# marvinli00/genie2

Measured on AMD Instinct MI355X. Metric: denoise-steps/sec (N=256, T=1000, batch=8), higher is better.
Workload: dtype f32 (pair-stack products as 3 f16 MFMAs on 2xf16-split operands, f32 accumulate); 1 GPU; unconditional N=256, T=1000, batch=8 per GPU, random-init base Denoiser (15.7M params), scale=0.6, reverse-loop steps 995..667; parallelism=replica per GPU x1, no data-path collective

## Files before the change

### genie2_amd/capi.py

```python
import ctypes as C
import os

import torch

_HERE = os.path.dirname(os.path.abspath(__file__))
LIB_PATH = os.environ.get('GENIE_HIP_LIB', os.path.join(_HERE, 'lib', 'libgenie_hip.so'))


class GenieDims(C.Structure):
    _fields_ = [
        ('c_s', C.c_int32), ('c_p', C.c_int32),
        ('c_pos_emb', C.c_int32), ('c_chain_emb', C.c_int32), ('c_timestep_emb', C.c_int32),
        ('relpos_k', C.c_int32),
        ('template_dist_n_bin', C.c_int32),
        ('template_dist_min', C.c_float), ('template_dist_step', C.c_float),
        ('n_pair_transform_layer', C.c_int32), ('c_hidden_mul', C.c_int32), ('pair_transition_n', C.c_int32),
        ('n_structure_layer', C.c_int32), ('n_structure_block', C.c_int32),
        ('c_hidden_ipa', C.c_int32), ('n_head_ipa', C.c_int32), ('n_qk_point', C.c_int32), ('n_v_point', C.c_int32),
        ('rescale', C.c_float),
        ('n_timestep', C.c_int32), ('max_n_res', C.c_int32), ('max_n_chain', C.c_int32),
    ]


class GenieFeatures(C.Structure):
    _fields_ = [(k, C.c_void_p) for k in (
        'aatype', 'atom_positions', 'residue_mask', 'residue_index', 'chain_index',
        'fixed_sequence_mask', 'fixed_structure_mask', 'interface_mask')]


class GenieTaps(C.Structure):
    _fields_ = [(k, C.c_void_p) for k in ('s', 'p', 's_final', 'rots_out', 'trans_out', 'p_init', 'p_layer0', 'states', 'p_trimul_out0',
                                              'ipa_cat0')]


class GenieGemmDesc(C.Structure):
    _fields_ = [(n, C.c_int32) for n in ('M', 'N', 'K', 'batch', 'nb2', 'nsplit', 'mode', 'terms', 'relu')] + \
               [(n, C.c_int64) for n in ('am', 'ak', 'bk', 'bn', 'cm', 'cn', 'a1', 'a2', 'b1', 'b2', 'c1', 'c2')] + [('alpha', C.c_float)] + \
               [('cblk', C.c_int32), ('cblk_m', C.c_int32), ('ctab', C.c_int64 * 8), ('atab', C.c_int64 * 8)]


class GenieTrainOpts(C.Structure):
    _fields_ = [('tri_dropout', C.c_float), ('ipa_dropout', C.c_float), ('transition_dropout', C.c_float), ('seed', C.c_uint32),
                ('train_mode', C.c_int32), ('fast_math', C.c_int32), ('struct_done_event', C.c_void_p)]


SYMBOLS = {
    'genie_create': (C.c_int, [C.POINTER(GenieDims), C.c_int, C.POINTER(C.c_void_p)]),
# ... 66 lines not shown
```

### genie2_amd/csrc/common.h

```cpp
#pragma once
#include <hip/hip_runtime.h>
#include <stdint.h>
#include "../../include/genie_hip.h"

typedef float f32x16 __attribute__((ext_vector_type(16)));
typedef float f32x4 __attribute__((ext_vector_type(4)));

#define GENIE_LN_EPS 1e-5f

#ifdef __HIPCC__

__device__ __forceinline__ f32x16 mfma_8k(const float4 a, const float4 b, f32x16 c) {
    c = __builtin_amdgcn_mfma_f32_32x32x2f32(a.x, b.x, c, 0, 0, 0);
    c = __builtin_amdgcn_mfma_f32_32x32x2f32(a.y, b.y, c, 0, 0, 0);
    c = __builtin_amdgcn_mfma_f32_32x32x2f32(a.z, b.z, c, 0, 0, 0);
    c = __builtin_amdgcn_mfma_f32_32x32x2f32(a.w, b.w, c, 0, 0, 0);
    return c;
}

__device__ __forceinline__ f32x16 zero16() {
    f32x16 z;
#pragma unroll
    for (int i = 0; i < 16; ++i) z[i] = 0.f;
    return z;
// ... 154 lines not shown
    char err[512];

    bool have_weights;
    float* wdev;
    bool hx;
    unsigned char* hxdev;
    HxGemmW hxg[64]; int n_hxg;
    unsigned hx_launches;
    size_t wdev_floats;
    float *single_w;
    float *pij_w;
    float *relpos_t;
    float *templ_w;
    float *motif_w;
    float *ipa_bias_w, *ipa_bias_b;
    PairLayerW* pair;
    StructLayerW* st;

    bool have_tables;
    float *pos_tab, *chain_tab, *t_tab, *sched;
    int n_pos, n_chain;
    float* sched_host;

    int B, N, NP;
    bool have_feats, has_motif;
    int32_t *f_aatype, *f_rmask, *f_ridx, *f_cidx;
    float *f_pos;
    uint8_t *f_fsm, *f_fstm, *f_ifm;
    float *rmaskf;

// ... 59 lines not shown
```

### genie2_amd/csrc/genie_api.hip

```cpp
#include <stdio.h>
#include <stdlib.h>
#include <string.h>
#include <math.h>
#include <algorithm>
#include <cmath>
#include <new>
#include <string>
#include <vector>

#include "common.h"

void pair_kernels_init();
void pair_fused_kernels_init();
void single_kernels_init(const genie_dims_t& d, int n_max);
void launch_scale_copy(genie_ctx* h, hipStream_t st, const float* in, float* out, int n, float s);
size_t ipa_attn_lds(const genie_dims_t& d, int N);

static char g_create_err[512] = "";

#define SET_ERR(h, ...) do { snprintf((h)->err, sizeof((h)->err), __VA_ARGS__); } while (0)
#define HIP_TRY(h, call) do { hipError_t e_ = (call); if (e_ != hipSuccess) { \
    SET_ERR(h, "%s failed: %s (%s:%d)", #call, hipGetErrorString(e_), __FILE__, __LINE__); return GENIE_E_HIP; } } while (0)

static const char* kKernelNames[KC_COUNT] = {
// ... 424 lines not shown
        auto w = vcat({{q_w, H * C * cs}, {kv_w, 2 * H * C * cs}, {qp_w, 3 * H * Pq * cs}, {kp_w, 3 * H * (Pq + Pv) * cs}});
        auto bv = vcat({{q_b, H * C}, {kv_b, 2 * H * C}, {qp_b, 3 * H * Pq}, {kp_b, 3 * H * (Pq + Pv)}});
        pack_gemm(&S.proj_w, w.data(), ipa_proj_n(d), (int)cs);
        slot(&S.proj_b, img.raw(bv.data(), bv.size()));
        wb_all.insert(wb_all.end(), b_w, b_w + H * cp);
        bb_all.insert(bb_all.end(), b_b, b_b + H);
        pack_gemm(&S.out_w, o_w, (int)cs, (int)ncat); slot(&S.out_b, img.raw(o_b, cs));
        slot(&S.ln_ipa_g, img.raw(li_g, cs)); slot(&S.ln_ipa_b, img.raw(li_b, cs));
        pack_gemm(&S.t1_w, t1w, (int)cs, (int)cs); slot(&S.t1_b, img.raw(t1b, cs));
        pack_gemm(&S.t2_w, t2w, (int)cs, (int)cs); slot(&S.t2_b, img.raw(t2b, cs));
        pack_gemm(&S.t3_w, t3w, (int)cs, (int)cs); slot(&S.t3_b, img.raw(t3b, cs));
        slot(&S.ln_tr_g, img.raw(lt_g, cs)); slot(&S.ln_tr_b, img.raw(lt_b, cs));
        slot(&S.bb_w, img.raw(bw, 6 * cs)); slot(&S.bb_b, img.raw(bbs, 6));
    }
    pack_gemm(&h->ipa_bias_w, wb_all.data(), (int)(d.n_structure_layer * H), (int)cp);
    slot(&h->ipa_bias_b, img.raw(bb_all.data(), bb_all.size()));
    if (c.left != 0) { SET_ERR(h, "genie_load_weights: %zu floats left over", c.left); return GENIE_E_ARG; }

    if (h->wdev) { (void)hipFree(h->wdev); h->wdev = nullptr; }
    img.add(64);
    HIP_TRY(h, hipMalloc((void**)&h->wdev, img.data.size() * sizeof(float)));
    HIP_TRY(h, hipMemcpy(h->wdev, img.data.data(), img.data.size() * sizeof(float), hipMemcpyHostToDevice));
    h->wdev_floats = img.data.size();
    for (auto& f : fix) *f.first = h->wdev + f.second;
    if (h->hxdev) { (void)hipFree(h->hxdev); h->hxdev = nullptr; }
    hx.begin();
    HIP_TRY(h, hipMalloc((void**)&h->hxdev, hx.d.size() * 2 + 256));
    HIP_TRY(h, hipMemcpy(h->hxdev, hx.d.data(), hx.d.size() * 2, hipMemcpyHostToDevice));
    for (auto& f : hxfix) *f.first = h->hxdev + f.second;
    h->n_hxg = 0;
// ... 131 lines not shown
    launch_gemm_rows(h, st, h->s0, cs, M, cs, h->pij_w, 2 * cp, nullptr, nullptr, 0, nullptr, 0, h->pij, 2 * cp);
    launch_pair_init(h, st, h->trans_w, h->rots_w, codes);
    if (taps && taps->p_init) HIP_TRY(h, d2d(taps->p_init, h->p, P * cp * 4));

    const bool fused = launch_pair_stack_fused(h, st, taps ? taps->p_trimul_out0 : nullptr, taps ? taps->p_layer0 : nullptr);
    for (int l = 0; l < (fused ? 0 : d.n_pair_transform_layer); ++l) {
        launch_trimul(h, st, h->pair[l].out, true);
        if (l == 0 && taps && taps->p_trimul_out0) HIP_TRY(h, d2d(taps->p_trimul_out0, h->p, P * cp * 4));
        launch_trimul(h, st, h->pair[l].in, false);
        launch_pair_transition(h, st, h->pair[l]);
        if (l == 0 && taps && taps->p_layer0) HIP_TRY(h, d2d(taps->p_layer0, h->p, P * cp * 4));
    }
    if (taps && taps->p) HIP_TRY(h, d2d(taps->p, h->p, P * cp * 4));

    launch_ipa_bias(h, st);
    HIP_TRY(h, d2d(h->s, h->s0, (size_t)M * cs * 4));
    if (taps && taps->states) HIP_TRY(h, d2d(taps->states, h->s0, (size_t)M * cs * 4));
    int n_state = 1;
    const int nproj = ipa_proj_n(d), ncat = ipa_cat_n(d);
    bool split = h->st2 && B >= 2 && M >= 1024 && ipa_attn_splits(h) && !getenv("GENIE_NO_STRUCT_SPLIT");
    for (int l = 0; split && l < d.n_structure_layer; ++l) split = struct_tail_fused(h, h->st[l]);
    const int n_half = split ? 2 : 1;
    const int n_layers = d.n_structure_block * d.n_structure_layer;
    hipStream_t hstream[2] = {st, h->st2};
    if (split) {
        HIP_TRY(h, hipEventRecord(h->ev_fork, st));
        HIP_TRY(h, hipStreamWaitEvent(h->st2, h->ev_fork, 0));
    }
    for (int half = 0; half < n_half; ++half) {
        hipStream_t hs = hstream[half];
// ... 168 lines not shown
```

### genie2_amd/csrc/hx_fused.h

```cpp
#pragma once
#include "hx_pair.h"

#define FZ_SB_BZ 0
#define FZ_SB_BG 128
#define FZ_SB_B1 256
#define FZ_SB_B2 768
#define FZ_SB_BP 896
#define FZ_SB_FLOATS 1408
#define FZ_OOR 0x7FFFFFF0
#ifndef FZ_SAFE
#define FZ_SAFE 0
#endif
#define FZ_FULL_WAIT(bit) do { if (FZ_SAFE & (bit)) asm volatile("s_waitcnt vmcnt(0) lgkmcnt(0)" ::: "memory"); else asm volatile("" ::: "memory"); } while (0)

struct FusedArgs {
    float* z; const float* xcm; const float* rmask; const unsigned char* wimg;
    const float *bzs, *bgs, *b1s, *b2s, *bproj;
    unsigned *acm, *bcm;
    int N, NP, n_wtiles, n_hb;
    unsigned cm_bytes, z_bytes;
    float sx, cgo, cz, c1, c2, inv_c2, cpa, cpb, cg;
    int rev, stagger;
};

__device__ __forceinline__ void fz_zt_read(float4 (&raw)[16], const unsigned char* zt, int pl, int h, int half) {
#pragma unroll
    for (int q = 0; q < 4; ++q) {
        const int g = 4 * q + h;
        raw[2 * (4 * half + q)] = *reinterpret_cast<const float4*>(zt + pl * 256 + ((g ^ (pl & 15)) << 4));
        raw[2 * (4 * half + q) + 1] = *reinterpret_cast<const float4*>(zt + pl * 256 + (((g + 2) ^ (pl & 15)) << 4));
    }
}

__device__ __forceinline__ void fz_zt_chunk(float4& a, float4& b, const unsigned char* zt, int pl, int h, int q) {
    const int g = 4 * q + h;
    a = *reinterpret_cast<const float4*>(zt + pl * 256 + ((g ^ (pl & 15)) << 4));
    b = *reinterpret_cast<const float4*>(zt + pl * 256 + (((g + 2) ^ (pl & 15)) << 4));
// ... 54 lines not shown
```

### genie2_amd/csrc/pair_fused_kernels.hip

```cpp
#include <string.h>
#include "hx_fused.h"

#define FZ_LDS_BYTES (2 * HX_STAGE_BYTES + 6144 + 8 * HX_ZT_BYTES)
#ifndef FZ_XPRE
#define FZ_XPRE 0
#endif
#ifndef FZ_ASYM
#define FZ_ASYM 1
#endif
#ifndef FZ_BIASPRE
#define FZ_BIASPRE 1
#endif
#ifndef FZ_KO
#define FZ_KO 0
#endif
#ifndef FZ_ZEARLY
#define FZ_ZEARLY 0
#endif

#ifdef FZ_TS
__device__ unsigned long long g_fz_ts[16][2048];
extern "C" int genie_fz_debug_read(unsigned long long* out) { return (int)hipMemcpyFromSymbol(out, HIP_SYMBOL(g_fz_ts), sizeof(unsigned long long) * 16 * 2048); }
#define FZ_TS_DECL() const bool ts_on = blockIdx.x == 0 && HAS_P;       unsigned long long* ts_p = g_fz_ts[(HAS_T ? 8 : 0) + (threadIdx.x >> 6)]; int ts_n = 0
#define FZ_STAMP() do { if (ts_on) { const unsigned long long t_ = __builtin_amdgcn_s_memtime(); if ((threadIdx.x & 63) == 0 && ts_n < 2048) ts_p[ts_n] = t_; ++ts_n; } } while (0)
#else
#define FZ_TS_DECL()
#define FZ_STAMP() do { } while (0)
#endif
#if defined(FZ_TS) && FZ_TS == 2
#define FZ_STAMP2() FZ_STAMP()
#else
#define FZ_STAMP2() do { } while (0)
#endif
#if defined(FZ_TS) && FZ_TS == 3
#define FZ_STAMP3() FZ_STAMP()
#else
#define FZ_STAMP3() do { } while (0)
#endif

template <bool COL, bool HAS_T, bool HAS_P = true>
__global__ __launch_bounds__(512, 1) void k_pair_fused(const FusedArgs A) {
    extern __shared__ __attribute__((aligned(16))) unsigned char smb[];
    float* sb = reinterpret_cast<float*>(smb + 2 * HX_STAGE_BYTES);
    const int lane = threadIdx.x & 63, wave = UNI(threadIdx.x >> 6);
    const int h = lane >> 5, pl = lane & 31;
    const int N = A.N, NP = A.NP, n_wtiles = A.n_wtiles;
    const int ntile = (N + 31) >> 5;
    const int n_tiles = (n_wtiles + 7) / 8;
    const int rev = A.rev;
    const int n_hb = HAS_T ? A.n_hb : 0;
    const int PBASE = 4 + n_hb;
    const rsrc_t rw = hx_rsrc(A.wimg, (unsigned)((PBASE + (HAS_P ? 8 : 0)) * HX_STAGE_BYTES));
    const rsrc_t rx = hx_rsrc(A.xcm, A.cm_bytes), rz = hx_rsrc(A.z, A.z_bytes);
    const rsrc_t ra = hx_rsrc(A.acm, A.cm_bytes), rb = hx_rsrc(A.bcm, A.cm_bytes);
    const int lane16 = lane * 16;
    const int sstride = NP * NP * 4;
    const int zstride = COL ? N * 512 : 512;
    auto issue = [&](int s, int buf) {
#if FZ_ASYM
        if (wave >= 4) {
#pragma unroll
            for (int q = 0; q < 8; ++q) {
                const int p = 8 * (wave - 4) + q;
                hx_dma(rw, smb + buf * HX_STAGE_BYTES + p * 1024, lane16, s * HX_STAGE_BYTES + p * 1024);
            }
        }
#else
#pragma unroll
        for (int q = 0; q < 4; ++q) {
            const int p = 4 * wave + q;
            hx_dma(rw, smb + buf * HX_STAGE_BYTES + p * 1024, lane16, s * HX_STAGE_BYTES + p * 1024);
        }
#endif
    };
    unsigned char* zt = smb + 2 * HX_STAGE_BYTES + 6144 + wave * HX_ZT_BYTES;
    auto tile_geom = [&](int tile, int& zsoff, int& nv, int& cmoff) {
        const int wt = min(HX_PHYS(tile) * 8 + wave, n_wtiles - 1);
        const int st = wt % ntile, line = (wt / ntile) % N, b = wt / (ntile * N);
        nv = min(32, N - st * 32);
        zsoff = COL ? ((b * N + st * 32) * N + line) * 512 : ((b * N + line) * N + st * 32) * 512;
        cmoff = ((b * 128 * NP + line) * NP + st * 32) * 4;
    };
    const int vx = (4 * h * NP * NP + pl) * 4;
#define FZ_XLOAD(c, xoff) do {                                                                                              \
        raw[2 * (c)].x = hx_load(rx, vx, (xoff) + (16 * (c) + 0) * sstride); raw[2 * (c)].y = hx_load(rx, vx, (xoff) + (16 * (c) + 1) * sstride); \
        raw[2 * (c)].z = hx_load(rx, vx, (xoff) + (16 * (c) + 2) * sstride); raw[2 * (c)].w = hx_load(rx, vx, (xoff) + (16 * (c) + 3) * sstride); \
// ... 9 lines not shown
    int tile = blockIdx.x;
    FZ_TS_DECL();
    if (A.stagger > 0) {
        const long long t0 = (long long)__builtin_amdgcn_s_memtime();
        const long long wait = (long long)A.stagger * ((blockIdx.x >> 3) & 7) / 8;
        while ((long long)__builtin_amdgcn_s_memtime() - t0 < wait) __builtin_amdgcn_s_sleep(8);
    }
    issue(0, 0);
    for (int u = threadIdx.x; u < FZ_SB_FLOATS; u += 512) {
        float v = 0.f;
        if (u < FZ_SB_BG) v = A.bzs[u];
        else if (u < FZ_SB_B1) v = A.bgs[u - FZ_SB_BG];
        else if (u < FZ_SB_B2) { if (HAS_T && u - FZ_SB_B1 < n_hb * 32) v = A.b1s[u - FZ_SB_B1]; }
        else if (u < FZ_SB_BP) { if (HAS_T) v = A.b2s[u - FZ_SB_B2]; }
        else if (HAS_P) v = A.bproj[u - FZ_SB_BP];
        sb[u] = v;
    }
    float4 raw[16];
    {
        int zs, nv, cm;
        tile_geom(tile, zs, nv, cm);
        if (HAS_T && FZ_XPRE) {
#pragma unroll
            for (int c = 0; c < 4; ++c) FZ_XLOAD(c, cm);
        }
        hx_zt_dma(rz, zt, lane, zs, zstride, nv, 1);
    }
    hx_stage_landed();
    __syncthreads();

#pragma unroll 1
    for (; tile < n_tiles; tile += gridDim.x) {
// ... 157 lines not shown
            fz_stats(v, A.sx, mean, sc);
            fz_split_tile(zh, zl, v, mean, sc);
#pragma unroll
            for (int ob = 0; ob < 4; ++ob)
#pragma unroll
                for (int r = 0; r < 16; ++r) v[ob][r] = fmaf(v[ob][r], A.inv_c2, sbt[FZ_SB_B2 + ob * 32 + acc_row(r, lane)]);
#if FZ_BIASPRE
            f32x16 d;
#pragma unroll
            for (int r = 0; r < 16; ++r) d[r] = sbt[FZ_SB_B1 + acc_row(r, lane)];
#endif
            auto t_stage = [&](int hb, auto xc_tag) {
                constexpr int XC = decltype(xc_tag)::value;
                if ((FZ_KO & 8) && hb + 1 < n_hb) { }
                else if (HAS_P || hb + 1 < n_hb) issue(4 + hb + 1, (hb + 1) & 1);
                else if (more) issue(0, 0);
                const unsigned char* stage = smb + (hb & 1) * HX_STAGE_BYTES;
#if !FZ_BIASPRE
                f32x16 d;
#pragma unroll
                for (int r = 0; r < 16; ++r) d[r] = sbt[FZ_SB_B1 + hb * 32 + acc_row(r, lane)];
#endif
                {
                    h8 wh = hx_frag(stage, 0, 0, lane), wl = hx_frag(stage, 0, 1, lane);
#pragma unroll
                    for (int kc = 0; kc < 8; ++kc) {
                        const h8 nh = (FZ_KO & 2) ? wh : hx_frag(stage, min(kc + 1, 7), 0, lane), nl = (FZ_KO & 2) ? wl : hx_frag(stage, min(kc + 1, 7), 1, lane);
                        PIPE_FENCE();
                        MFH3(wh, wl, zh[kc], zl[kc], d);
                        PIPE_FENCE();
// ... 40 lines not shown
            for (int hb = 0; hb < n_plain; ++hb) t_stage(hb, std::integral_constant<int, -1>{});
            if (FZ_XPRE && n_hb >= 4) {
                t_stage(n_hb - 4, std::integral_constant<int, 0>{});
                t_stage(n_hb - 3, std::integral_constant<int, 1>{});
                t_stage(n_hb - 2, std::integral_constant<int, 2>{});
                t_stage(n_hb - 1, std::integral_constant<int, 3>{});
            }
            FZ_STAMP();
            const float m2 = msk * A.c2;
#pragma unroll
            for (int ob = 0; ob < 4; ++ob)
#pragma unroll
                for (int r = 0; r < 16; ++r) v[ob][r] *= m2;
        }

        fz_store_half(rz, zt, v[0], v[1], lane_t, zsoff, zstride, nvalid, 0);
        FZ_FULL_WAIT(128);
        FZ_STAMP3();
        fz_store_half(rz, zt, v[2], v[3], lane_t, zsoff, zstride, nvalid, 1);
        FZ_FULL_WAIT(64);
        FZ_STAMP3();
        if constexpr (HAS_P) {
            float mean, sc;
            fz_stats(v, A.sx, mean, sc);
            fz_split_tile(zh, zl, v, mean, sc);
        }
        hx_lds_done();
        FZ_STAMP();
        if constexpr (!HAS_P) {
            if (more) hx_zt_dma(rz, zt, lane_t, n_zsoff, zstride, n_nv, 1);
        }

        if constexpr (HAS_P) {
            const float* sbias = sbt + FZ_SB_BP;
            const float cg = A.cg;
            const float ma = msk * A.cpa, mb = msk * A.cpb;
            const int voff = (pl < nvalid) ? (4 * h * NP * NP + pl) * 4 : FZ_OOR;
            const int sbase = ((b * 128 * NP + line) * NP + t0i) * 4;
            unsigned wst[8];
            f32x16 apA, agA, apB, agB;
#pragma unroll
            for (int r = 0; r < 16; ++r) { apB[r] = 0.f; agB[r] = 0.f; apA[r] = sbias[acc_row(r, lane)]; agA[r] = sbias[256 + acc_row(r, lane)]; }
#pragma unroll 1
            for (int pp = 0; pp < 4; ++pp) {
                {
// ... 39 lines not shown
                const int e_voff = voff, e_so = sbase + 3 * 32 * sstride;
                const float e_pm = mb;
                float t[16], u[16];
#pragma unroll
                for (int r = 0; r < 16; ++r) {
                    HX_PROJ_PIECE_A(agB, r, t[r]);
                    HX_PROJ_PIECE_B(apB, r, t[r], u[r]);
                }
                PIPE_FENCE();
#pragma unroll
                for (int r = 0; r < 16; ++r) HX_PROJ_PIECE_C_NOW(r, t[r], u[r]);
            }
            FZ_STAMP();
        }
    }
#undef FZ_XLOAD
}

static int fz_num_cu() {
    static int n = 0;
    if (!n) { int dev = 0; hipDeviceProp_t pr; (void)hipGetDevice(&dev); (void)hipGetDeviceProperties(&pr, dev); n = pr.multiProcessorCount > 0 ? pr.multiProcessorCount : 256; }
    return n;
}

void pair_fused_kernels_init() {
    (void)hipFuncSetAttribute(reinterpret_cast<const void*>(k_pair_fused<true, false>), hipFuncAttributeMaxDynamicSharedMemorySize, FZ_LDS_BYTES);
    (void)hipFuncSetAttribute(reinterpret_cast<const void*>(k_pair_fused<false, true>), hipFuncAttributeMaxDynamicSharedMemorySize, FZ_LDS_BYTES);
    (void)hipFuncSetAttribute(reinterpret_cast<const void*>(k_pair_fused<false, true, false>), hipFuncAttributeMaxDynamicSharedMemorySize, FZ_LDS_BYTES);
}

void launch_pair_fused(genie_ctx* h, hipStream_t st, const HxFusedW& f, const HxTriW& o, const HxTransW* t, const HxTriW* pp, bool col) {
    const HxTriW& p = pp ? *pp : o;
    const int N = h->N, NP = h->NP, ntile = (N + 31) / 32;
    FusedArgs a;
    a.z = h->p; a.xcm = h->xcm; a.rmask = h->rmaskf; a.wimg = f.img;
    a.bzs = o.bzs; a.bgs = o.bgs; a.b1s = t ? t->b1s : nullptr; a.b2s = t ? t->b2s : nullptr; a.bproj = p.bias_proj;
    a.acm = reinterpret_cast<unsigned*>(h->acm); a.bcm = reinterpret_cast<unsigned*>(h->bcm);
    a.N = N; a.NP = NP; a.n_wtiles = h->B * N * ntile; a.n_hb = t ? h->d.pair_transition_n * 4 : 0;
    a.cm_bytes = (unsigned)((size_t)h->B * 128 * NP * NP * 4);
    a.z_bytes = (unsigned)((size_t)h->B * N * N * 512);
    a.sx = o.sx; a.cgo = o.cgo; a.cz = o.cz;
    a.c1 = t ? t->c1 : 0.f; a.c2 = t ? t->c2 : 1.f; a.inv_c2 = t ? 1.0f / t->c2 : 1.f;
    a.cpa = p.cpa; a.cpb = p.cpb; a.cg = p.cg;
    a.rev = (int)(h->hx_launches++ & 1);
    { static const int stagger = [] { const char* e = getenv("GENIE_FZ_STAGGER"); return e ? atoi(e) : 0; }(); a.stagger = stagger; }
    const long long n_tiles = ((long long)a.n_wtiles + 7) / 8;
    const unsigned grid = (unsigned)(n_tiles < fz_num_cu() ? n_tiles : fz_num_cu());
    if (!pp) hipLaunchKernelGGL((k_pair_fused<false, true, false>), dim3(grid), dim3(512), FZ_LDS_BYTES, st, a);
    else if (col) hipLaunchKernelGGL((k_pair_fused<true, false>), dim3(grid), dim3(512), FZ_LDS_BYTES, st, a);
    else hipLaunchKernelGGL((k_pair_fused<false, true>), dim3(grid), dim3(512), FZ_LDS_BYTES, st, a);
}
```

### genie2_amd/csrc/pair_hx_kernels.hip

```cpp
#include "hx_pair.h"


template <int NW>
__global__ __launch_bounds__(NW * 64, NW == 8 ? 1 : 2) void k_pair_transition_hx(
    float* __restrict__ z, const float* __restrict__ rmask, const unsigned char* __restrict__ wimg,
    const float* __restrict__ b1s, const float* __restrict__ b2s, int N, long long M, int n_hb, float sx, float c1, float c2, int rev) {
    extern __shared__ __attribute__((aligned(16))) unsigned char smb[];
    float* sb1 = reinterpret_cast<float*>(smb + 2 * HX_STAGE_BYTES);
    const int lane = threadIdx.x & 63, wave = UNI(threadIdx.x >> 6);
    const int h = lane >> 5, pl = lane & 31;
    const int n_wt = (int)((M + 31) / 32);
    const int n_tiles = (n_wt + NW - 1) / NW;
    const rsrc_t rw = hx_rsrc(wimg, (unsigned)(n_hb * HX_STAGE_BYTES));
    const rsrc_t rz = hx_rsrc(z, (unsigned)(M * 512));
    const rsrc_t rnull = hx_rsrc(z, 0u);
    const int lane16 = lane * 16;
    constexpr int PW = 32 / NW;
    auto issue = [&](int hb, int buf) {
#pragma unroll
        for (int q = 0; q < PW; ++q) {
            const int p = PW * wave + q;
            hx_dma(rw, smb + buf * HX_STAGE_BYTES + p * 1024, lane16, hb * HX_STAGE_BYTES + p * 1024);
        }
    };
// ... 889 lines not shown
    const bool resident = getenv("GENIE_OUT_STREAMED") == nullptr;
    if (resident)
        hipLaunchKernelGGL(k_trimul_out_hx_r<8>, dim3(hx_grid((g.n_wt + 7) / 8, 8, v.cus)), dim3(512), 4 * HX_STAGE_BYTES, st, g.zs, g.xcm,
                           x.img_out, x.bgs, x.bzs, g.N, g.NP, g.n_wt, g.cm_bytes, g.z_bytes, x.sx, x.cgo, x.cz, (int)(v.launches++ & 1));
    else
        hipLaunchKernelGGL(k_trimul_out_hx<8>, dim3(hx_grid((g.n_wt + 7) / 8, 8, v.cus)), dim3(512), HX_LDS_BYTES, st, g.zs, g.xcm, x.img_out,
                           x.bgs, x.bzs, g.N, g.NP, g.n_wt, g.cm_bytes, g.z_bytes, x.sx, x.cgo, x.cz, (int)(v.launches++ & 1));
}

static void trimul_slice(genie_ctx* h, HxSlice& v, const TriMulW& w, bool outgoing) {
    trimul_proj_slice(h, v, w, outgoing);
    trimul_contract_slice(h, v, w, false);
    trimul_out_slice(h, v, w);
}

void launch_pair_fused(genie_ctx* h, hipStream_t st, const HxFusedW& f, const HxTriW& o, const HxTransW* t, const HxTriW* p, bool col);
bool launch_pair_stack_fused(genie_ctx* h, hipStream_t st, float* tap_trimul_out0, float* tap_layer0) {
    const int L = h->d.n_pair_transform_layer;
    if (!h->hx || L < 1 || getenv("GENIE_NO_PAIR_FUSE") || (getenv("GENIE_HX_SLICE") && atoi(getenv("GENIE_HX_SLICE")) > 0)) return false;
    if ((h->d.pair_transition_n * 4) & 1) return false;
    const size_t pbytes = (size_t)h->B * h->N * h->N * h->d.c_p * 4;
    HxSlice v{0, h->B, st, hx_num_cu(), h->hx_launches, h->prof};
    trimul_proj_slice(h, v, h->pair[0].out, true);
    for (int l = 0; l < L; ++l) {
        const PairLayerW& W = h->pair[l];
        trimul_contract_slice(h, v, W.out, true);
        h->hx_launches = v.launches;
        { ProfScope ps(h, st, KC_PAIR_FUSED_A); launch_pair_fused(h, st, W.fa, W.out.hx, nullptr, &W.in.hx, true); }
        v.launches = h->hx_launches;
        if (l == 0 && tap_trimul_out0) (void)hipMemcpyAsync(tap_trimul_out0, h->p, pbytes, hipMemcpyDeviceToDevice, st);
        trimul_contract_slice(h, v, W.in, false);
        if (l + 1 < L) {
            h->hx_launches = v.launches;
            { ProfScope ps(h, st, KC_PAIR_FUSED_B); launch_pair_fused(h, st, W.fb, W.in.hx, &W.hx_pt, &h->pair[l + 1].out.hx, false); }
            v.launches = h->hx_launches;
        } else {
            h->hx_launches = v.launches;
            { ProfScope ps(h, st, KC_PAIR_FUSED_B); launch_pair_fused(h, st, W.fb, W.in.hx, &W.hx_pt, nullptr, false); }
            v.launches = h->hx_launches;
        }
        if (l == 0 && tap_layer0) (void)hipMemcpyAsync(tap_layer0, h->p, pbytes, hipMemcpyDeviceToDevice, st);
    }
    h->hx_launches = v.launches;
    return true;
}

void launch_pair_transition_hx(genie_ctx* h, hipStream_t st, const PairLayerW& w) {
    HxSlice v{0, h->B, st, hx_num_cu(), h->hx_launches, h->prof};
    pair_transition_slice(h, v, w);
    h->hx_launches = v.launches;
}

static int g_hx_slice = 0;
// ... 71 lines not shown
            for (int blk = 0; blk < 3; ++blk)
#pragma unroll
                for (int r = 0; r < 16; ++r) {
                    const int o = blk * 32 + (r & 3) + 8 * (r >> 2) + 4 * hf;
                    if (o < LH) out[((((size_t)o * B + b) * N + i) * N) + j0 + n] = fmaf(acc[blk][r], isc, sbias[o]);
                }
        }
    }
#pragma unroll
    for (int o = 32; o > 0; o >>= 1) amax = fmaxf(amax, __shfl_xor(amax, o));
    if (lane == 0 && __float_as_uint(amax) > *reinterpret_cast<volatile unsigned*>(pmax)) atomicMax(pmax, __float_as_uint(amax));
}

bool launch_ipa_bias_hx(genie_ctx* h, hipStream_t st) {
    const int LH = h->d.n_structure_layer * h->d.n_head_ipa;
    if (!h->hx || LH > 96 || h->d.c_p != 128 || getenv("GENIE_IPA_BIAS_F32")) return false;
    const HxGemmW* w = nullptr;
    for (int i = 0; i < h->n_hxg; ++i)
        if (h->hxg[i].w == h->ipa_bias_w) w = &h->hxg[i];
    if (!w) return false;
    const int N = h->N, n_tiles = h->B * N * ((N + 31) / 32);
    const int grid = n_tiles / 4 < 2 * hx_num_cu() ? (n_tiles + 3) / 4 : 2 * hx_num_cu();
    (void)hipMemsetAsync(h->pmax, 0, sizeof(unsigned), st);
    hipLaunchKernelGGL(k_ipa_bias_hx, dim3(grid), dim3(256), IB_UNITS * 2048 + 96 * 4, st, h->p, w->img, w->inv_s, h->ipa_bias_b, h->ipa_bias,
                       h->B, N, LH, n_tiles, (int)(h->hx_launches & 1), h->pmax);
    return true;
}

void pair_hx_kernels_init() {
#define HX_ATTR(k) (void)hipFuncSetAttribute(reinterpret_cast<const void*>(k), hipFuncAttributeMaxDynamicSharedMemorySize, HX_LDS_BYTES)
    HX_ATTR((k_trimul_proj_hx<true, 8>)); HX_ATTR((k_trimul_proj_hx<false, 8>));
// ... 7 lines not shown
```

### genie2_amd/csrc/pair_kernels.hip

```cpp
#include "common.h"

#define LDZ 132


template <bool AMAX = false>
__device__ __forceinline__ float load_tile64(float* tile, const float* __restrict__ src, size_t row_stride,
                                             int nvalid, int tid) {
    const int c4 = tid & 31;
    const int r0 = tid >> 5;
    float4 v[8];
    const int last = max(nvalid - 1, 0);
#pragma unroll
    for (int u = 0; u < 8; ++u) {
        const int r = min(r0 + 8 * u, last);
        v[u] = *reinterpret_cast<const float4*>(src + (size_t)r * row_stride + c4 * 4);
    }
#pragma unroll
    for (int u = 0; u < 8; ++u) {
        const int r = r0 + 8 * u;
        if (r >= nvalid) v[u] = make_float4(0.f, 0.f, 0.f, 0.f);
        *reinterpret_cast<float4*>(tile + r * LDZ + c4 * 4) = v[u];
    }
    float am = 0.f;
    if constexpr (AMAX) {
// ... 416 lines not shown
    {
        ProfScope ps(h, st, KC_TRIMUL_OUT);
        launch_trimul_out_wl(h, st, w);
    }
}

void launch_pair_transition_hx(genie_ctx* h, hipStream_t st, const PairLayerW& w);
void launch_pair_transition(genie_ctx* h, hipStream_t st, const PairLayerW& w) {
    ProfScope ps(h, st, KC_PAIR_TRANSITION);
    if (h->hx) launch_pair_transition_hx(h, st, w);
    else launch_pair_transition_wl(h, st, w);
}

bool launch_ipa_bias_hx(genie_ctx* h, hipStream_t st);
void launch_ipa_bias(genie_ctx* h, hipStream_t st) {
    ProfScope ps(h, st, KC_IPA_BIAS);
    if (launch_ipa_bias_hx(h, st)) return;
    const int N = h->N, ntile = (N + 127) / 128;
    const int LH = h->d.n_structure_layer * h->d.n_head_ipa;
    const size_t lds = 128 * LDZ * sizeof(float);
    (void)hipMemsetAsync(h->pmax, 0, sizeof(unsigned), st);
    hipLaunchKernelGGL(k_ipa_bias, dim3(h->B * N * ntile), dim3(256), lds, st, h->p, h->ipa_bias_w, h->ipa_bias_b, h->ipa_bias,
                       h->B, N, LH, h->hx ? (int)(h->hx_launches & 1) : 0, h->pmax);
}

void pair_wl_kernels_init();
void pair_hx_kernels_init();
void pair_kernels_init() {
    pair_wl_kernels_init();
    pair_hx_kernels_init();
// ... 6 lines not shown
```

### genie2_amd/engine.py

```python
import ctypes as C

import torch

from . import capi, pack

_FEATURE_DTYPES = {
    'aatype': torch.int32, 'atom_positions': torch.float32, 'residue_mask': torch.int32,
    'residue_index': torch.int32, 'chain_index': torch.int32,
    'fixed_sequence_mask': torch.bool, 'fixed_structure_mask': torch.bool, 'interface_mask': torch.bool,
}


def _ptr(t):
    return C.c_void_p(t.data_ptr()) if t is not None else C.c_void_p(0)


def adam_step(p, g, m, v, lr, step, betas=(0.9, 0.999), eps=1e-8):
    lib = capi.load_library()
    for t in (p, g, m, v):
        assert t.is_cuda and t.dtype == torch.float32 and t.is_contiguous() and t.numel() == p.numel()
    rc = lib.genie_adam_step(C.c_void_p(torch.cuda.current_stream(p.device).cuda_stream), p.numel(), _ptr(p), _ptr(g), _ptr(m), _ptr(v),
                             float(lr), float(betas[0]), float(betas[1]), float(eps), int(step))
    if rc != 0:
        raise capi.GenieError('genie_adam_step failed (%d)' % rc)
# ... 145 lines not shown
            rc = self.lib.genie_denoise_vjp(self._h, self._stream(), _ptr(w), _ptr(tr), _ptr(ro), _ptr(ts), _ptr(codes), _ptr(g), _ptr(z), _ptr(dt))
        capi.check(self._h, rc, 'genie_denoise_vjp')
        return z, dt

    def denoise(self, trans, rots, timesteps, quat_codes=None, taps=()):
        B, N = self.B, self.N
        trans = self._dev(trans, torch.float32)
        rots = self._dev(rots, torch.float32)
        ts = self._dev(timesteps, torch.int32)
        codes = self._dev(quat_codes, torch.int8) if quat_codes is not None else None
        z = torch.empty(B, N, 3, device=self.device)
        shapes = {'s': (B, N, self.dims['c_s']), 'p': (B, N, N, self.dims['c_p']), 's_final': (B, N, self.dims['c_s']),
                  'rots_out': (B, N, 3, 3), 'trans_out': (B, N, 3), 'p_init': (B, N, N, self.dims['c_p']),
                  'p_layer0': (B, N, N, self.dims['c_p']), 'p_trimul_out0': (B, N, N, self.dims['c_p']),
                  'ipa_cat0': (B, N, self.dims['n_head_ipa'] * (self.dims['c_hidden_ipa'] + 4 * self.dims['n_v_point'] + self.dims['c_p'])),
                  'states': (1 + self.dims['n_structure_block'] * self.dims['n_structure_layer'], B, N, self.dims['c_s'])}
        out = {k: torch.empty(shapes[k], device=self.device) for k in taps}
        ct = capi.GenieTaps(**{k: v.data_ptr() for k, v in out.items()})
        rc = self.lib.genie_denoise(self._h, self._stream(), _ptr(trans), _ptr(rots), _ptr(ts), _ptr(codes), _ptr(z),
                                    C.byref(ct) if taps else None)
        capi.check(self._h, rc, 'genie_denoise')
        out['z'] = z
        return out

    def p_sample(self, step, scale, trans, z, eps):
        rots = torch.empty(self.B, self.N, 3, 3, device=self.device)
        rc = self.lib.genie_p_sample(self._h, self._stream(), int(step), float(scale), _ptr(trans), _ptr(rots), _ptr(z),
                                     _ptr(eps))
        capi.check(self._h, rc, 'genie_p_sample')
        return rots

# ... 30 lines not shown
```

### include/genie_hip.h

```cpp
#ifndef GENIE_HIP_H
#define GENIE_HIP_H

#include <stddef.h>
#include <stdint.h>

#ifdef __cplusplus
extern "C" {
#endif

#define GENIE_OK            0
#define GENIE_E_ARG        -1
#define GENIE_E_STATE      -2
#define GENIE_E_HIP        -3
#define GENIE_E_NOMEM      -4

typedef struct genie_ctx* genie_handle_t;
typedef void* genie_stream_t;

typedef struct {
    int32_t c_s, c_p;
    int32_t c_pos_emb, c_chain_emb, c_timestep_emb;
    int32_t relpos_k;
    int32_t template_dist_n_bin;
    float   template_dist_min, template_dist_step;
// ... 14 lines not shown
    const uint8_t* fixed_structure_mask;
    const uint8_t* interface_mask;
} genie_features_t;

typedef struct {
    float* s;
    float* p;
    float* s_final;
    float* rots_out;
    float* trans_out;
    float* p_init;
    float* p_layer0;
    float* states;
    float* p_trimul_out0;
    float* ipa_cat0;
} genie_taps_t;


int genie_create(const genie_dims_t* dims, int device, genie_handle_t* out);
void genie_destroy(genie_handle_t h);
const char* genie_last_error(genie_handle_t h);

size_t genie_weight_count(const genie_dims_t* dims);

int genie_load_weights(genie_handle_t h, const float* blob, size_t n_floats);

int genie_set_tables(genie_handle_t h, const float* pos_tab, int n_pos,
                     const float* chain_tab, int n_chain,
                     const float* t_tab, const float* sched);

// ... 85 lines not shown
```

Before: 106.3 batch-steps/s.

## Fuse IPA pair-bias projection and pair abs-max into last fused pair kernel

Computes the IPA attention bias projection (pair features times per-head weights, plus bias) inside the last fused pair-stack kernel while the final pair tile is still in registers. The same pass produces the pair abs-max through LDS and global atomics. The standalone ipa_bias launch is then skipped, which saves a full re-read of the pair tensor. In exchange the last pair kernel gets extra weight DMA stages, MFMA work, barriers and scattered stores, and the fused path has its own per-tile fp16 split scaling that can differ numerically from the standalone path.

Measured after the change: 107.0 batch-steps/s (median of 6 runs). No clear change (+0.6%).

```diff
diff --git a/genie2_amd/capi.py b/genie2_amd/capi.py
--- a/genie2_amd/capi.py
+++ b/genie2_amd/capi.py
@@ -30,7 +30,7 @@
 
 class GenieTaps(C.Structure):
     _fields_ = [(k, C.c_void_p) for k in ('s', 'p', 's_final', 'rots_out', 'trans_out', 'p_init', 'p_layer0', 'states', 'p_trimul_out0',
-                                              'ipa_cat0')]
+                                              'ipa_cat0', 'ipa_bias', 'pmax')]
 
 
 class GenieGemmDesc(C.Structure):
diff --git a/genie2_amd/csrc/common.h b/genie2_amd/csrc/common.h
--- a/genie2_amd/csrc/common.h
+++ b/genie2_amd/csrc/common.h
@@ -192,6 +192,9 @@
     float *templ_w;
     float *motif_w;
     float *ipa_bias_w, *ipa_bias_b;
+    const unsigned char* ipa_bias_fimg;
+    float ipa_bias_finv;
+    bool ipa_bias_done;
     PairLayerW* pair;
     StructLayerW* st;
 
diff --git a/genie2_amd/csrc/genie_api.hip b/genie2_amd/csrc/genie_api.hip
--- a/genie2_amd/csrc/genie_api.hip
+++ b/genie2_amd/csrc/genie_api.hip
@@ -462,6 +462,18 @@
         slot(&S.bb_w, img.raw(bw, 6 * cs)); slot(&S.bb_b, img.raw(bbs, 6));
     }
     pack_gemm(&h->ipa_bias_w, wb_all.data(), (int)(d.n_structure_layer * H), (int)cp);
+    h->ipa_bias_fimg = nullptr;
+    if (d.n_structure_layer * H <= 96 && cp == 128) {
+        const int LH = (int)(d.n_structure_layer * H);
+        const float sw = p2floor(16384.0 / max_abs(wb_all.data(), (size_t)LH * cp));
+        h->ipa_bias_finv = 1.0f / sw;
+        hxfix.push_back({&h->ipa_bias_fimg, hx.begin()});
+        for (int blk = 0; blk < 4; ++blk)
+            for (int kc = 0; kc < 8; ++kc)
+                hx.unit([&](int i, int hh, int e) {
+                    const int r = 32 * blk + i;
+                    return r < LH ? wb_all[(size_t)r * cp + 16 * kc + (e & 3) + 8 * (e >> 2) + 4 * hh] * sw : 0.f; });
+    }
     slot(&h->ipa_bias_b, img.raw(bb_all.data(), bb_all.size()));
     if (c.left != 0) { SET_ERR(h, "genie_load_weights: %zu floats left over", c.left); return GENIE_E_ARG; }
 
@@ -623,6 +635,8 @@
     if (taps && taps->p) HIP_TRY(h, d2d(taps->p, h->p, P * cp * 4));
 
     launch_ipa_bias(h, st);
+    if (taps && taps->ipa_bias) HIP_TRY(h, d2d(taps->ipa_bias, h->ipa_bias, (size_t)d.n_structure_layer * d.n_head_ipa * P * 4));
+    if (taps && taps->pmax) HIP_TRY(h, d2d(taps->pmax, reinterpret_cast<const float*>(h->pmax), 4));
     HIP_TRY(h, d2d(h->s, h->s0, (size_t)M * cs * 4));
     if (taps && taps->states) HIP_TRY(h, d2d(taps->states, h->s0, (size_t)M * cs * 4));
     int n_state = 1;
diff --git a/genie2_amd/csrc/hx_fused.h b/genie2_amd/csrc/hx_fused.h
--- a/genie2_amd/csrc/hx_fused.h
+++ b/genie2_amd/csrc/hx_fused.h
@@ -21,6 +21,9 @@
     unsigned cm_bytes, z_bytes;
     float sx, cgo, cz, c1, c2, inv_c2, cpa, cpb, cg;
     int rev, stagger;
+    unsigned ib_off; const float* ibias; float* ibout; unsigned* pmax;
+    int B, LH;
+    float ibinv;
 };
 
 __device__ __forceinline__ void fz_zt_read(float4 (&raw)[16], const unsigned char* zt, int pl, int h, int half) {
diff --git a/genie2_amd/csrc/pair_fused_kernels.hip b/genie2_amd/csrc/pair_fused_kernels.hip
--- a/genie2_amd/csrc/pair_fused_kernels.hip
+++ b/genie2_amd/csrc/pair_fused_kernels.hip
@@ -38,7 +38,7 @@
 #define FZ_STAMP3() do { } while (0)
 #endif
 
-template <bool COL, bool HAS_T, bool HAS_P = true>
+template <bool COL, bool HAS_T, bool HAS_P = true, bool HAS_IB = false>
 __global__ __launch_bounds__(512, 1) void k_pair_fused(const FusedArgs A) {
     extern __shared__ __attribute__((aligned(16))) unsigned char smb[];
     float* sb = reinterpret_cast<float*>(smb + 2 * HX_STAGE_BYTES);
@@ -50,26 +50,28 @@
     const int rev = A.rev;
     const int n_hb = HAS_T ? A.n_hb : 0;
     const int PBASE = 4 + n_hb;
-    const rsrc_t rw = hx_rsrc(A.wimg, (unsigned)((PBASE + (HAS_P ? 8 : 0)) * HX_STAGE_BYTES));
+    const rsrc_t rw = hx_rsrc(A.wimg, HAS_IB ? A.ib_off + 2 * HX_STAGE_BYTES : (unsigned)((PBASE + (HAS_P ? 8 : 0)) * HX_STAGE_BYTES));
     const rsrc_t rx = hx_rsrc(A.xcm, A.cm_bytes), rz = hx_rsrc(A.z, A.z_bytes);
     const rsrc_t ra = hx_rsrc(A.acm, A.cm_bytes), rb = hx_rsrc(A.bcm, A.cm_bytes);
+    const rsrc_t rio = hx_rsrc(A.ibout, HAS_IB ? (unsigned)((size_t)A.LH * A.B * N * N * 4) : 0u);
     const int lane16 = lane * 16;
     const int sstride = NP * NP * 4;
     const int zstride = COL ? N * 512 : 512;
-    auto issue = [&](int s, int buf) {
+    auto issue = [&](int s, int buf, bool ib = false) {
+        const int base = ib ? (int)A.ib_off : 0;
 #if FZ_ASYM
         if (wave >= 4) {
 #pragma unroll
             for (int q = 0; q < 8; ++q) {
                 const int p = 8 * (wave - 4) + q;
-                hx_dma(rw, smb + buf * HX_STAGE_BYTES + p * 1024, lane16, s * HX_STAGE_BYTES + p * 1024);
+                hx_dma(rw, smb + buf * HX_STAGE_BYTES + p * 1024, lane16, base + s * HX_STAGE_BYTES + p * 1024);
             }
         }
 #else
 #pragma unroll
         for (int q = 0; q < 4; ++q) {
             const int p = 4 * wave + q;
-            hx_dma(rw, smb + buf * HX_STAGE_BYTES + p * 1024, lane16, s * HX_STAGE_BYTES + p * 1024);
+            hx_dma(rw, smb + buf * HX_STAGE_BYTES + p * 1024, lane16, base + s * HX_STAGE_BYTES + p * 1024);
         }
 #endif
     };
@@ -109,8 +111,11 @@
         else if (u < FZ_SB_B2) { if (HAS_T && u - FZ_SB_B1 < n_hb * 32) v = A.b1s[u - FZ_SB_B1]; }
         else if (u < FZ_SB_BP) { if (HAS_T) v = A.b2s[u - FZ_SB_B2]; }
         else if (HAS_P) v = A.bproj[u - FZ_SB_BP];
+        else if (HAS_IB && u - FZ_SB_BP < A.LH) v = A.ibias[u - FZ_SB_BP];
         sb[u] = v;
     }
+    unsigned* lds_amax = reinterpret_cast<unsigned*>(sb + FZ_SB_FLOATS);
+    if (HAS_IB && threadIdx.x == 0) *lds_amax = 0u;
     float4 raw[16];
     {
         int zs, nv, cm;
@@ -298,6 +303,7 @@
                 constexpr int XC = decltype(xc_tag)::value;
                 if ((FZ_KO & 8) && hb + 1 < n_hb) { }
                 else if (HAS_P || hb + 1 < n_hb) issue(4 + hb + 1, (hb + 1) & 1);
+                else if (HAS_IB) issue(0, 0, true);
                 else if (more) issue(0, 0);
                 const unsigned char* stage = smb + (hb & 1) * HX_STAGE_BYTES;
 #if !FZ_BIASPRE
@@ -368,6 +374,7 @@
                 for (int r = 0; r < 16; ++r) v[ob][r] *= m2;
         }
 
+        if constexpr (HAS_IB) issue(1, 1, true);
         fz_store_half(rz, zt, v[0], v[1], lane_t, zsoff, zstride, nvalid, 0);
         FZ_FULL_WAIT(128);
         FZ_STAMP3();
@@ -383,6 +390,59 @@
         FZ_STAMP();
         if constexpr (!HAS_P) {
             if (more) hx_zt_dma(rz, zt, lane_t, n_zsoff, zstride, n_nv, 1);
+        }
+
+        if constexpr (HAS_IB) {
+            float m = 0.f;
+#pragma unroll
+            for (int ob = 0; ob < 4; ++ob)
+#pragma unroll
+                for (int r = 0; r < 16; ++r) m = fmaxf(m, fabsf(v[ob][r]));
+            m = fmaxf(m, __shfl_xor(m, 32));
+            {
+                float wm = m;
+#pragma unroll
+                for (int o = 16; o > 0; o >>= 1) wm = fmaxf(wm, __shfl_xor(wm, o));
+                if (lane == 0) atomicMax(lds_amax, __float_as_uint(wm));
+            }
+            const int e = (int)((__builtin_bit_cast(unsigned, m) >> 23) & 255u);
+            const bool tiny = e < 16;
+            const float sc = tiny ? 1.0f : __builtin_bit_cast(float, (unsigned)(268 - e) << 23);
+            const float isc = (tiny ? 1.0f : __builtin_bit_cast(float, (unsigned)(e - 14) << 23)) * A.ibinv;
+            hx_stage_landed();
+            hx_stage_barrier();
+            f32x16 ib[3];
+#pragma unroll
+            for (int k = 0; k < 3; ++k) ib[k] = zero16();
+#pragma unroll
+            for (int kc = 0; kc < 8; ++kc) {
+                float x[8];
+#pragma unroll
+                for (int q = 0; q < 8; ++q) x[q] = v[kc >> 1][8 * (kc & 1) + q];
+                h8 ph, plo;
+                hx_split8(x, sc, ph, plo);
+                const h8 f0 = hx_frag(smb, kc, 0, lane), f0l = hx_frag(smb, kc, 1, lane);
+                const h8 f1 = hx_frag(smb, 8 + kc, 0, lane), f1l = hx_frag(smb, 8 + kc, 1, lane);
+                const h8 f2 = hx_frag(smb + HX_STAGE_BYTES, kc, 0, lane), f2l = hx_frag(smb + HX_STAGE_BYTES, kc, 1, lane);
+                MFH3(f0, f0l, ph, plo, ib[0]);
+                MFH3(f1, f1l, ph, plo, ib[1]);
+                MFH3(f2, f2l, ph, plo, ib[2]);
+            }
+            hx_stage_barrier();
+            if (more) issue(0, 0);
+            const int P = A.B * N * N;
+            const int vo = (4 * h_t * P + (b * N + line) * N + t0i + pl_t) * 4;
+#pragma unroll
+            for (int k = 0; k < 3; ++k)
+#pragma unroll
+                for (int r = 0; r < 16; ++r) {
+                    const int o0 = 32 * k + (r & 3) + 8 * (r >> 2);
+                    const bool ok = pl_t < nvalid && o0 + 4 * h_t < A.LH;
+                    hx_store(rio, fmaf(ib[k][r], isc, sbt[FZ_SB_BP + acc_row(r, lane_t) + 32 * k]), ok ? vo + o0 * P * 4 : FZ_OOR, 0);
+                }
+            asm volatile("s_waitcnt vmcnt(48)" ::: "memory");
+            __builtin_amdgcn_sched_barrier(0);
+            hx_stage_barrier();
         }
 
         if constexpr (HAS_P) {
@@ -452,6 +512,10 @@
             FZ_STAMP();
         }
     }
+    if constexpr (HAS_IB) {
+        __syncthreads();
+        if (threadIdx.x == 0 && *lds_amax > *reinterpret_cast<volatile unsigned*>(A.pmax)) atomicMax(A.pmax, *lds_amax);
+    }
 #undef FZ_XLOAD
 }
 
@@ -465,9 +529,10 @@
     (void)hipFuncSetAttribute(reinterpret_cast<const void*>(k_pair_fused<true, false>), hipFuncAttributeMaxDynamicSharedMemorySize, FZ_LDS_BYTES);
     (void)hipFuncSetAttribute(reinterpret_cast<const void*>(k_pair_fused<false, true>), hipFuncAttributeMaxDynamicSharedMemorySize, FZ_LDS_BYTES);
     (void)hipFuncSetAttribute(reinterpret_cast<const void*>(k_pair_fused<false, true, false>), hipFuncAttributeMaxDynamicSharedMemorySize, FZ_LDS_BYTES);
+    (void)hipFuncSetAttribute(reinterpret_cast<const void*>(k_pair_fused<false, true, false, true>), hipFuncAttributeMaxDynamicSharedMemorySize, FZ_LDS_BYTES);
 }
 
-void launch_pair_fused(genie_ctx* h, hipStream_t st, const HxFusedW& f, const HxTriW& o, const HxTransW* t, const HxTriW* pp, bool col) {
+void launch_pair_fused(genie_ctx* h, hipStream_t st, const HxFusedW& f, const HxTriW& o, const HxTransW* t, const HxTriW* pp, bool col, bool ib) {
     const HxTriW& p = pp ? *pp : o;
     const int N = h->N, NP = h->NP, ntile = (N + 31) / 32;
     FusedArgs a;
@@ -482,9 +547,12 @@
     a.cpa = p.cpa; a.cpb = p.cpb; a.cg = p.cg;
     a.rev = (int)(h->hx_launches++ & 1);
     { static const int stagger = [] { const char* e = getenv("GENIE_FZ_STAGGER"); return e ? atoi(e) : 0; }(); a.stagger = stagger; }
+    a.ib_off = ib ? (unsigned)(h->ipa_bias_fimg - f.img) : 0u; a.ibias = h->ipa_bias_b; a.ibout = h->ipa_bias; a.pmax = h->pmax;
+    a.B = h->B; a.LH = h->d.n_structure_layer * h->d.n_head_ipa; a.ibinv = h->ipa_bias_finv;
     const long long n_tiles = ((long long)a.n_wtiles + 7) / 8;
     const unsigned grid = (unsigned)(n_tiles < fz_num_cu() ? n_tiles : fz_num_cu());
-    if (!pp) hipLaunchKernelGGL((k_pair_fused<false, true, false>), dim3(grid), dim3(512), FZ_LDS_BYTES, st, a);
+    if (!pp && ib) hipLaunchKernelGGL((k_pair_fused<false, true, false, true>), dim3(grid), dim3(512), FZ_LDS_BYTES, st, a);
+    else if (!pp) hipLaunchKernelGGL((k_pair_fused<false, true, false>), dim3(grid), dim3(512), FZ_LDS_BYTES, st, a);
     else if (col) hipLaunchKernelGGL((k_pair_fused<true, false>), dim3(grid), dim3(512), FZ_LDS_BYTES, st, a);
     else hipLaunchKernelGGL((k_pair_fused<false, true>), dim3(grid), dim3(512), FZ_LDS_BYTES, st, a);
 }
diff --git a/genie2_amd/csrc/pair_hx_kernels.hip b/genie2_amd/csrc/pair_hx_kernels.hip
--- a/genie2_amd/csrc/pair_hx_kernels.hip
+++ b/genie2_amd/csrc/pair_hx_kernels.hip
@@ -927,9 +927,14 @@
     trimul_out_slice(h, v, w);
 }
 
-void launch_pair_fused(genie_ctx* h, hipStream_t st, const HxFusedW& f, const HxTriW& o, const HxTransW* t, const HxTriW* p, bool col);
+void launch_pair_fused(genie_ctx* h, hipStream_t st, const HxFusedW& f, const HxTriW& o, const HxTransW* t, const HxTriW* p, bool col,
+                       bool ib = false);
+static bool ipa_bias_hx_applies(const genie_ctx* h) {
+    return h->hx && h->d.n_structure_layer * h->d.n_head_ipa <= 96 && h->d.c_p == 128 && !getenv("GENIE_IPA_BIAS_F32");
+}
 bool launch_pair_stack_fused(genie_ctx* h, hipStream_t st, float* tap_trimul_out0, float* tap_layer0) {
     const int L = h->d.n_pair_transform_layer;
+    h->ipa_bias_done = false;
     if (!h->hx || L < 1 || getenv("GENIE_NO_PAIR_FUSE") || (getenv("GENIE_HX_SLICE") && atoi(getenv("GENIE_HX_SLICE")) > 0)) return false;
     if ((h->d.pair_transition_n * 4) & 1) return false;
     const size_t pbytes = (size_t)h->B * h->N * h->N * h->d.c_p * 4;
@@ -948,8 +953,11 @@
             { ProfScope ps(h, st, KC_PAIR_FUSED_B); launch_pair_fused(h, st, W.fb, W.in.hx, &W.hx_pt, &h->pair[l + 1].out.hx, false); }
             v.launches = h->hx_launches;
         } else {
+            const bool ib = h->ipa_bias_fimg && ipa_bias_hx_applies(h);
+            if (ib) (void)hipMemsetAsync(h->pmax, 0, sizeof(unsigned), st);
             h->hx_launches = v.launches;
-            { ProfScope ps(h, st, KC_PAIR_FUSED_B); launch_pair_fused(h, st, W.fb, W.in.hx, &W.hx_pt, nullptr, false); }
+            { ProfScope ps(h, st, KC_PAIR_FUSED_B); launch_pair_fused(h, st, W.fb, W.in.hx, &W.hx_pt, nullptr, false, ib); }
+            h->ipa_bias_done = ib;
             v.launches = h->hx_launches;
         }
         if (l == 0 && tap_layer0) (void)hipMemcpyAsync(tap_layer0, h->p, pbytes, hipMemcpyDeviceToDevice, st);
@@ -1051,7 +1059,7 @@
 
 bool launch_ipa_bias_hx(genie_ctx* h, hipStream_t st) {
     const int LH = h->d.n_structure_layer * h->d.n_head_ipa;
-    if (!h->hx || LH > 96 || h->d.c_p != 128 || getenv("GENIE_IPA_BIAS_F32")) return false;
+    if (!ipa_bias_hx_applies(h)) return false;
     const HxGemmW* w = nullptr;
     for (int i = 0; i < h->n_hxg; ++i)
         if (h->hxg[i].w == h->ipa_bias_w) w = &h->hxg[i];
diff --git a/genie2_amd/csrc/pair_kernels.hip b/genie2_amd/csrc/pair_kernels.hip
--- a/genie2_amd/csrc/pair_kernels.hip
+++ b/genie2_amd/csrc/pair_kernels.hip
@@ -454,6 +454,7 @@
 
 bool launch_ipa_bias_hx(genie_ctx* h, hipStream_t st);
 void launch_ipa_bias(genie_ctx* h, hipStream_t st) {
+    if (h->ipa_bias_done) { h->ipa_bias_done = false; return; }
     ProfScope ps(h, st, KC_IPA_BIAS);
     if (launch_ipa_bias_hx(h, st)) return;
     const int N = h->N, ntile = (N + 127) / 128;
diff --git a/genie2_amd/engine.py b/genie2_amd/engine.py
--- a/genie2_amd/engine.py
+++ b/genie2_amd/engine.py
@@ -183,7 +183,8 @@
                   'rots_out': (B, N, 3, 3), 'trans_out': (B, N, 3), 'p_init': (B, N, N, self.dims['c_p']),
                   'p_layer0': (B, N, N, self.dims['c_p']), 'p_trimul_out0': (B, N, N, self.dims['c_p']),
                   'ipa_cat0': (B, N, self.dims['n_head_ipa'] * (self.dims['c_hidden_ipa'] + 4 * self.dims['n_v_point'] + self.dims['c_p'])),
-                  'states': (1 + self.dims['n_structure_block'] * self.dims['n_structure_layer'], B, N, self.dims['c_s'])}
+                  'states': (1 + self.dims['n_structure_block'] * self.dims['n_structure_layer'], B, N, self.dims['c_s']),
+                  'ipa_bias': (self.dims['n_structure_layer'] * self.dims['n_head_ipa'], B, N, N), 'pmax': (1,)}
         out = {k: torch.empty(shapes[k], device=self.device) for k in taps}
         ct = capi.GenieTaps(**{k: v.data_ptr() for k, v in out.items()})
         rc = self.lib.genie_denoise(self._h, self._stream(), _ptr(trans), _ptr(rots), _ptr(ts), _ptr(codes), _ptr(z),
diff --git a/include/genie_hip.h b/include/genie_hip.h
--- a/include/genie_hip.h
+++ b/include/genie_hip.h
@@ -52,6 +52,8 @@
     float* states;
     float* p_trimul_out0;
     float* ipa_cat0;
+    float* ipa_bias;
+    float* pmax;
 } genie_taps_t;
 
 
```
